# turian/inverse-audio-synthesis

Hardware: AMD Instinct MI355X
Metric: audio-seconds rendered+lossed/sec (whole node), batch=128 4s@44.1kHz (higher is better)
Workload: dtype f32; 1 GPU; BASELINE configs[1]: torchsynth-style Voice render + PQMF(3) analysis + mel-L1 loss, batch 128 x 4 s @ 44100 Hz per GPU; batch_per_gpu=128, samples_per_voice=176400, launch=hipgraph, streams=5, pipelined=True

## Files before the change

inverse-audio-synthesis_amd/csrc/voice_kernels.hip:

```cpp
#include <cstdio>
#include <cstdlib>
#include "voice_math.h"
#include "wave_ops.h"
#include "voice_trig.h"
#include "voice_table.h"

#define VOICE_THREADS 256
#define VOICE_WAVES (VOICE_THREADS / 64)
#define AUDIO_THREADS 256
#define AUDIO_WAVES (AUDIO_THREADS / 64)
#define VOICE_SPT 16
#define VOICE_TILE (AUDIO_THREADS * VOICE_SPT)

__constant__ IasParamRange c_param_table[IAS_NPARAMS] = IAS_PARAM_TABLE_INIT;


__device__ __forceinline__ float mapped_param(const float* __restrict__ params01, int b, int idx) {
  const IasParamRange r = c_param_table[idx];
  return ias_map_param(params01[(size_t)b * IAS_NPARAMS + idx], (float)r.lo, (float)r.span, (float)r.curve,
                       r.symmetric);
}

__device__ __forceinline__ int adsr_base(int a) {
  switch (a) {
// ... 133 lines not shown
  __shared__ float s_head[12];
  __shared__ float s_mode[2][8];
  __shared__ double s_wtot[2][CTLF_LFO_WAVES];
  const int b = blockIdx.x, tid = threadIdx.x, lane = tid & 63, wave = tid >> 6;
  const float eps = (float)IAS_EPS;

  for (int i = tid; i < IAS_CTL_TAB_DOUBLES; i += CTLF_THREADS) s_tab[i] = g_ctl_tab[i];
  if (tid < IAS_NPARAMS) s_p[tid] = mapped_param(params01, b, tid);
  __syncthreads();
  const float note_on = s_p[IAS_P_KEYBOARD_DURATION];
  if (wave == CTLF_WAVES - 1) {
    if (lane < 12) {
      const int a = lane >> 1;
      const float* q = s_p + adsr_base(a);
      IasAdsr e; e.attack = q[0]; e.decay = q[1]; e.sustain = q[2]; e.release = q[3]; e.alpha = q[4];
      const IasAdsrHeads h = ias_adsr_heads(e, note_on, control_rate, eps, s_tab);
      s_head[lane] = (lane & 1) ? h.release_head : h.decay_head;
    }
  } else if (wave == CTLF_WAVES - 2) {
    if (lane < 16 && (lane & 7) < 5) {
      const int l = lane >> 3, k = lane & 7;
      const int qbase = (l == 0) ? IAS_P_LFO_1_FREQUENCY : IAS_P_LFO_2_FREQUENCY;
      s_mode[l][k] = ias_pow_ctl(s_p[qbase + 3 + k], IAS_LFO_EXPONENT_F, s_tab);
    }
  } else if (wave == CTLF_WAVES - 3) {
    if (lane == 0) {
      const float* p = s_p;
      const float midi_f0 = p[IAS_P_KEYBOARD_MIDI_F0];
      IasVoiceConst vc;
      vc.f0_1 = ias_add(midi_f0, p[IAS_P_VCO_1_TUNING]);
      vc.depth_1 = p[IAS_P_VCO_1_MOD_DEPTH];
      vc.phi_1 = p[IAS_P_VCO_1_INITIAL_PHASE];
      vc.f0_2 = ias_add(midi_f0, p[IAS_P_VCO_2_TUNING]);
      vc.depth_2 = p[IAS_P_VCO_2_MOD_DEPTH];
      vc.phi_2 = p[IAS_P_VCO_2_INITIAL_PHASE];
      vc.kpart = ias_partials_k(midi_f0, vc.depth_2);
      vc.shape = p[IAS_P_VCO_2_SHAPE];
      vc.shape_gain = ias_sub(1.0f, ias_div(vc.shape, 2.0f));
      vc.lvl0 = p[IAS_P_MIXER_VCO_1];
      vc.lvl1 = p[IAS_P_MIXER_VCO_2];
      vc.lvl2 = p[IAS_P_MIXER_NOISE];
      vc.pad[0] = vc.pad[1] = vc.pad[2] = vc.pad[3] = 0.0f;
      vconst[b] = vc;
    }
  }
  __syncthreads();

  float* gsig = sig + (size_t)b * 8 * Tc;
  for (int idx = tid; idx < 6 * Tc; idx += CTLF_THREADS) {
    const int slot = idx / Tc, t = idx - slot * Tc;
    const int a = slot < 4 ? slot + 2 : slot - 4;
    const float* q = s_p + adsr_base(a);
    IasAdsr e; e.attack = q[0]; e.decay = q[1]; e.sustain = q[2]; e.release = q[3]; e.alpha = q[4];
    IasAdsrHeads heads; heads.decay_head = s_head[2 * a]; heads.release_head = s_head[2 * a + 1];
    const float v = ias_adsr_headed(t, e, note_on, control_rate, eps, heads, s_tab);
    s_row[a * Tc + t] = v;
    gsig[a * Tc + t] = v;
  }
  if (tid < 2) {
    float* m = s_mode[tid];
    const float sm = (float)((double)m[0] + (double)m[1] + (double)m[2] + (double)m[3] + (double)m[4]);
    for (int k = 0; k < 5; ++k) m[k] = ias_div(m[k], sm);
  }
  __syncthreads();

  {
    const int l = wave / CTLF_LFO_WAVES, w = wave - l * CTLF_LFO_WAVES;
    const int qbase = (l == 0) ? IAS_P_LFO_1_FREQUENCY : IAS_P_LFO_2_FREQUENCY;
    const float freq = s_p[qbase], depth = s_p[qbase + 1], phi = s_p[qbase + 2];
    const float* rate_env = s_row + (4 + l) * Tc;
    const float* amp_env = s_row + (2 + l) * Tc;
    double* sums = s_sum + (size_t)l * Tc;
    const int per_wave = ((Tc + CTLF_LFO_WAVES - 1) / CTLF_LFO_WAVES + 63) / 64 * 64;
    const int t_begin = min(w * per_wave, Tc), t_end = min(t_begin + per_wave, Tc);
    double carry = 0.0;
    for (int t0 = t_begin; t0 < t_end; t0 += 64) {
      const int t = t0 + lane;
      double inc = 0.0;
      if (t < t_end) inc = (double)ias_lfo_inc(freq, depth, rate_env[t], control_rate);
      const double sc = wave_incl_scan(inc, lane) + carry;
      carry = __shfl(sc, 63, 64);
      if (t < t_end) sums[t] = sc;
    }
    if (lane == 0) s_wtot[l][w] = carry;
    __syncthreads();
    double base = 0.0;
    for (int k = 0; k < w; ++k) base += s_wtot[l][k];
    float mode[5];
#pragma unroll
    for (int k = 0; k < 5; ++k) mode[k] = s_mode[l][k];
    for (int t = t_begin + lane; t < t_end; t += 64) {
      const double ph = base + sums[t];
      const float arg = ias_add((float)ph, phi);
      const float o = ias_mul(ias_lfo_shape_mix(arg, mode, s_tab), amp_env[t]);
      s_row[(6 + l) * Tc + t] = o;
      gsig[(6 + l) * Tc + t] = o;
      if (dbg != nullptr) {
        dbg[((size_t)b * 10 + 6 + l) * Tc + t] = arg;
        dbg[((size_t)b * 10 + 8 + l) * Tc + t] = o;
      }
    }
  }
  __syncthreads();

  float* out = ctrl + (size_t)b * IAS_NCTRL * Tc;
  const float* wm = s_p + IAS_P_MOD_MATRIX_ADSR_1_TO_VCO_1_PITCH;
  for (int t = tid; t < Tc; t += CTLF_THREADS) {
    const float e0 = s_row[t], e1 = s_row[Tc + t], l0 = s_row[6 * Tc + t], l1 = s_row[7 * Tc + t];
#pragma unroll
    for (int j = 0; j < IAS_NCTRL; ++j)
      out[j * Tc + t] = ias_dot4_cr(wm[j], wm[5 + j], wm[10 + j], wm[15 + j], e0, e1, l0, l1);
    if (dbg != nullptr) {
#pragma unroll
      for (int r = 0; r < 6; ++r) dbg[((size_t)b * 10 + r) * Tc + t] = s_row[r * Tc + t];
    }
  }
}
static size_t voice_control_fused_lds(int Tc) {
  return sizeof(double) * (IAS_CTL_TAB_DOUBLES + 2 * (size_t)Tc) + sizeof(float) * 8 * (size_t)Tc;
}

#endif

#define VOICE_MAXCTRL 320
#define VOICE_SPIN_LIMIT (1u << 24)
#ifndef VOICE_SPIN_SLEEP
#define VOICE_SPIN_SLEEP 8
#endif
#define VOICE_READY_BIT 0x8000000000000000ull
#ifndef VOICE_MIN_WAVES
#define VOICE_MIN_WAVES 3
#endif
#ifndef VOICE_GROUP
#define VOICE_GROUP 4
#endif
#ifndef VOICE_NCOUNTERS
#define VOICE_NCOUNTERS 8
#endif
#define VOICE_SYNC_HEAD_BYTES ((VOICE_NCOUNTERS + 1) * 128)
#define VOICE_MATH_CR 0
#define VOICE_TAB_DOUBLES ((IAS_EXP2_TAB_LEN + 1) / 2 * 2)
#define VOICE_MATH_HW 1

typedef __attribute__((address_space(1))) unsigned long long gu64;
typedef __attribute__((address_space(1))) unsigned int gu32;

__device__ const double g_exp2_tab[IAS_EXP2_TAB_LEN] = IAS_EXP2_TAB_INIT;

#ifdef VOICE_STAMPS
__device__ unsigned long long* g_voice_stamps = nullptr;
extern "C" int ias_voice_debug_set_stamps(unsigned long long* p) {
  return hipMemcpyToSymbol(HIP_SYMBOL(g_voice_stamps), &p, sizeof(p)) == hipSuccess ? 0 : -3;
}
#define VSTAMP(slot) do { if (g_voice_stamps && have_cur && lane == 0) { unsigned long long* sp_ = g_voice_stamps + ((size_t)(cur.b * ntiles + cur.tile) * 4 + wave) * 12; sp_[slot] = __builtin_amdgcn_s_memtime(); if ((slot) == 0) sp_[10] = __builtin_amdgcn_s_memrealtime(); if ((slot) == 6) sp_[11] = __builtin_amdgcn_s_memrealtime(); } } while (0)
#else
#define VSTAMP(slot) do {} while (0)
#endif

typedef __attribute__((address_space(3))) void voice_lds_void;
typedef const __attribute__((address_space(3))) char voice_lds_cchar;
typedef float voice_f2 __attribute__((ext_vector_type(2)));
typedef const __attribute__((address_space(3))) voice_f2 voice_lds_cfloat2;
typedef const __attribute__((address_space(3))) double voice_lds_cdouble;

__device__ __forceinline__ float voice_exp2_cr_lds(float t, unsigned tab_biased) {
  const float u = fmaf(t, 256.0f, 12582912.0f);
  const float mf = u - 12582912.0f;
  const float r = fmaf(mf, -0.00390625f, t);
  const double tv = *(voice_lds_cdouble*)(uintptr_t)(tab_biased + ((unsigned)__float_as_uint(u) << 3));
  const double rd = (double)r;
  double p = IAS_EXP2_C4;
  p = fma(p, rd, IAS_EXP2_C3);
  p = fma(p, rd, IAS_EXP2_C2);
  p = fma(p, rd, IAS_EXP2_C1);
  p = fma(p, rd, 1.0);
  return (float)(p * tv);
}
typedef const __attribute__((address_space(1))) void voice_glb_void;
__device__ __forceinline__ voice_lds_cchar* voice_ctrl_row(float real, unsigned ctrl_biased) {
  unsigned addr;
  const int k = (int)real;
  asm("v_mad_u32_u24 %0, %1, 40, %2" : "=v"(addr) : "v"(k), "s"(ctrl_biased));
  return (voice_lds_cchar*)(uintptr_t)addr;
}
static_assert(IAS_NCTRL * 8 == 40, "voice_ctrl_row: the row stride is an immediate");
__device__ __forceinline__ float voice_lerp(float w0, float w1, voice_f2 q) { return fmaf(w0, q.x, w1 * q.y); }
template <int MATH, bool FMA_DIV>
__device__ __forceinline__ float voice_inc(float f0, float depth, float pm, unsigned tab_biased, double inv_sample_rate,
                                           float sr_f, float sr_r) {
  float c = f0 + depth * pm;
  c = fminf(fmaxf(c, 0.0f), 127.0f);
  const float t = ias_div_fma(c - 69.0f, 12.0f, 1.0f / 12.0f);
  const float e = (MATH == VOICE_MATH_CR) ? voice_exp2_cr_lds(t, tab_biased) : __builtin_amdgcn_exp2f(t);
  const float w = (float)IAS_TWO_PI_D * (440.0f * e);
  return FMA_DIV ? ias_div_fma(w, sr_f, sr_r) : ias_div_by_recip(w, inv_sample_rate);
}

#define VOICE_CTRL_ROW (IAS_NCTRL * 8)

__device__ __forceinline__ int voice_take_ticket(unsigned int* counters, int& c, int& tried, int ntiles, int nvoices) {
  while (tried < VOICE_NCOUNTERS) {
    const int nv_c = (nvoices - c + VOICE_NCOUNTERS - 1) / VOICE_NCOUNTERS;
    const unsigned n = __hip_atomic_fetch_add((gu32*)(counters + c * 32), 1u, __ATOMIC_RELAXED, __HIP_MEMORY_SCOPE_AGENT);
    if ((int)n < nv_c * ntiles) return (c << 24) | (int)n;
    c = (c + 1) % VOICE_NCOUNTERS;
    ++tried;
  }
  return -1;
}
struct VoiceTile {
  int tile, b, j_tile, c_lo, ncp;
  bool fast;
};
__device__ __forceinline__ VoiceTile voice_tile_of(int ticket, int nvoices, int T, int Tc, float scale) {
  VoiceTile t;
  const int c = ticket >> 24, n = ticket & 0xffffff;
  const int nv_c = (nvoices - c + VOICE_NCOUNTERS - 1) / VOICE_NCOUNTERS;
  t.tile = n / nv_c;
  t.b = (n - t.tile * nv_c) * VOICE_NCOUNTERS + c;
  t.j_tile = t.tile * VOICE_TILE;
  const int j_last = min(t.j_tile + VOICE_TILE, T) - 1;
  int i0, i1; float w0, w1;
  ias_interp_pos(t.j_tile, scale, Tc, i0, i1, w0, w1);
  t.c_lo = i0;
  ias_interp_pos(j_last, scale, Tc, i0, i1, w0, w1);
  t.ncp = i1 - t.c_lo + 1;
  t.fast = (t.j_tile + VOICE_TILE <= T) && (T & 3) == 0;
  return t;
}
__device__ __forceinline__ void voice_stage_ctrl(char* dst, const float* __restrict__ ctrl, const VoiceTile& t, int Tc) {
  const float* cb = ctrl + (size_t)t.b * IAS_NCTRL * Tc;
  for (int i = threadIdx.x; i < IAS_NCTRL * t.ncp; i += AUDIO_THREADS) {
    const int k = i / t.ncp, c = i - k * t.ncp;
    const float* crow = cb + k * Tc;
    reinterpret_cast<float2*>(dst)[c * IAS_NCTRL + k] = make_float2(crow[t.c_lo + c], crow[min(t.c_lo + c + 1, Tc - 1)]);
  }
}

template <int MATH, bool FMA_DIV, bool FAST>
__device__ __forceinline__ void voice_phase_a(const char* s_ctrl, const double* s_tab_, const IasVoiceConst& vc,
                                              const VoiceTile& t, int T, double inv_sample_rate, float sr_f, float sr_r,
                                              float scale, float (&inc1)[VOICE_SPT], float (&inc2)[VOICE_SPT],
                                              double& ex1, double& ex2, double (*wsum)[AUDIO_WAVES]) {
  const int tid = threadIdx.x, lane = tid & 63, wave = tid >> 6;
  const int j0 = t.j_tile + tid * VOICE_SPT;
  const float jf0 = (float)j0;
  const unsigned ctrl_biased = (unsigned)(uintptr_t)(voice_lds_cchar*)s_ctrl - (unsigned)(t.c_lo * VOICE_CTRL_ROW);
  const unsigned s_tab = (unsigned)(uintptr_t)(voice_lds_cchar*)s_tab_ - (0x4B400000u + (unsigned)IAS_EXP2_TAB_MIN) * 8u;
  double tot1 = 0.0, tot2 = 0.0;
#pragma unroll
  for (int e = 0; e < VOICE_SPT; ++e) {
    const float real = scale * (jf0 + (float)e);
    const float w1 = __builtin_amdgcn_fractf(real), w0 = 1.0f - w1;
    voice_lds_cchar* cp = voice_ctrl_row(real, ctrl_biased);
    const voice_f2 q1 = *(voice_lds_cfloat2*)cp, q2 = *(voice_lds_cfloat2*)(cp + 16);
    const float pm1 = voice_lerp(w0, w1, q1), pm2 = voice_lerp(w0, w1, q2);
    float a = voice_inc<MATH, FMA_DIV>(vc.f0_1, vc.depth_1, pm1, s_tab, inv_sample_rate, sr_f, sr_r);
    float d = voice_inc<MATH, FMA_DIV>(vc.f0_2, vc.depth_2, pm2, s_tab, inv_sample_rate, sr_f, sr_r);
    if (!FAST && j0 + e >= T) { a = 0.0f; d = 0.0f; }
    inc1[e] = a; inc2[e] = d;
    tot1 += (double)a; tot2 += (double)d;
    if ((e & (VOICE_GROUP - 1)) == VOICE_GROUP - 1) __builtin_amdgcn_sched_barrier(0);
  }
  const double in1 = wave_incl_scan(tot1, lane), in2 = wave_incl_scan(tot2, lane);
  if (lane == 63) { wsum[0][wave] = in1; wsum[1][wave] = in2; }
  ex1 = in1 - tot1; ex2 = in2 - tot2;
}

template <bool FAST>
__device__ __forceinline__ void voice_phase_b(const char* s_ctrl, float* s_stage, const IasVoiceConst& vc, const VoiceTile& t,
                                              const float* __restrict__ nrow, float* __restrict__ arow, int T, float scale,
                                              const float (&inc1)[VOICE_SPT], const float (&inc2)[VOICE_SPT], double ex1,
                                              double ex2, const double* s_carry, const double (*wsum)[AUDIO_WAVES],
                                              float& pk) {
  const int tid = threadIdx.x, lane = tid & 63;
  const int wave_u = __builtin_amdgcn_readfirstlane(tid >> 6);
  const int j0 = t.j_tile + tid * VOICE_SPT;
  float jf0 = (float)j0;
  asm volatile("" : "+v"(jf0));
  float* stage = s_stage + wave_u * (64 * VOICE_SPT);
  const int j_wave = t.j_tile + wave_u * (64 * VOICE_SPT);
  const int perm = (lane >> 2) & 3;
  const unsigned ctrl_biased = (unsigned)(uintptr_t)(voice_lds_cchar*)s_ctrl - (unsigned)(t.c_lo * VOICE_CTRL_ROW);

  const float kexp = -1.4426950408889634f * vc.kpart;
  double run1 = s_carry[0] + ex1, run2 = s_carry[1] + ex2;
  for (int w = 0; w < wave_u; ++w) { run1 += wsum[0][w]; run2 += wsum[1][w]; }
  float o[4], nz[4];
  float4 nz_next = make_float4(0.f, 0.f, 0.f, 0.f);
  auto load_noise4 = [&](int jq) -> float4 {
    return make_float4(jq < T ? nrow[jq] : 0.0f, jq + 1 < T ? nrow[jq + 1] : 0.0f, jq + 2 < T ? nrow[jq + 2] : 0.0f,
                       jq + 3 < T ? nrow[jq + 3] : 0.0f);
  };
  if (!FAST) nz_next = load_noise4(j0);
#pragma unroll
  for (int e = 0; e < VOICE_SPT; ++e) {
    if ((e & 3) == 0) {
      if (FAST) {
        const float4 v = *reinterpret_cast<const float4*>(stage + lane * VOICE_SPT + 4 * ((e >> 2) ^ perm));
        nz[0] = v.x; nz[1] = v.y; nz[2] = v.z; nz[3] = v.w;
      } else {
        nz[0] = nz_next.x; nz[1] = nz_next.y; nz[2] = nz_next.z; nz[3] = nz_next.w;
        if (e + 4 < VOICE_SPT) nz_next = load_noise4(j0 + e + 4);
      }
    }
    const float real = scale * (jf0 + (float)e);
    const float w1 = __builtin_amdgcn_fractf(real);
    voice_lds_cchar* cp = voice_ctrl_row(real, ctrl_biased);
    const voice_f2 qa = *(voice_lds_cfloat2*)(cp + 8), qb = *(voice_lds_cfloat2*)(cp + 24), qn = *(voice_lds_cfloat2*)(cp + 32);
    const float amp1 = fmaf(w1, qa.y, qa.x), amp2 = fmaf(w1, qb.y, qb.x), ampn = fmaf(w1, qn.y, qn.x);
    run1 += (double)inc1[e]; run2 += (double)inc2[e];
    const float arg1 = (float)run1 + vc.phi_1, arg2 = (float)run2 + vc.phi_2;
    float s2, c2, sgn;
    voice_sincos_sgn(arg2, s2, c2, sgn);
    const float th = voice_tanh_half_of_exp2arg(kexp * s2);
    const float v2 = th * fmaf(vc.shape, c2, sgn);
    float om = voice_cos(arg1) * amp1;
    om = fmaf(v2, amp2, om);
    om = fmaf(nz[e & 3], ampn, om);
    if (FAST || j0 + e < T) pk = fmaxf(pk, fabsf(om));
    o[e & 3] = om;
    if ((e & 3) == 3) {
      if (FAST) {
        *reinterpret_cast<float4*>(stage + lane * VOICE_SPT + 4 * ((e >> 2) ^ perm)) = make_float4(o[0], o[1], o[2], o[3]);
      } else {
        const int jq = j0 + e - 3;
#pragma unroll
        for (int x = 0; x < 4; ++x) if (jq + x < T) arow[jq + x] = o[x];
      }
      if ((e & (VOICE_GROUP - 1)) == VOICE_GROUP - 1) __builtin_amdgcn_sched_barrier(0);
    }
  }
  if (FAST) {
    const int dst = 4 * (lane ^ (lane >> 4));
#pragma unroll
    for (int q = 0; q < VOICE_SPT / 4; ++q)
      *reinterpret_cast<float4*>(arow + j_wave + q * 256 + dst) = *reinterpret_cast<const float4*>(stage + q * 256 + lane * 4);
  }
}

__device__ __forceinline__ float2 voice_ctrl_elem(const float* __restrict__ ctrl, const VoiceTile& t, int Tc, int i) {
  const int k = i / t.ncp, c = i - k * t.ncp;
  const float* crow = ctrl + ((size_t)t.b * IAS_NCTRL + k) * Tc;
  return make_float2(crow[t.c_lo + c], crow[min(t.c_lo + c + 1, Tc - 1)]);
}
__device__ __forceinline__ void voice_ctrl_put(char* dst, const VoiceTile& t, int i, float2 v, const IasVoiceConst& vc) {
  const int k = i / t.ncp, c = i - k * t.ncp;
  if (k == 1 || k == 3 || k == 4) {
    const float g = k == 1 ? vc.lvl0 : (k == 3 ? vc.lvl1 * vc.shape_gain : vc.lvl2);
    const float a = g * v.x;
    v = make_float2(a, g * v.y - a);
  }
  reinterpret_cast<float2*>(dst)[c * IAS_NCTRL + k] = v;
}

#define VOICE_WAVE_LOOKBACK (AUDIO_WAVES - 1)
#define VOICE_WAVE_PUBLISH (AUDIO_WAVES - 2)
template <int MATH, bool FMA_DIV>
__global__ __launch_bounds__(AUDIO_THREADS, VOICE_MIN_WAVES) __attribute__((amdgpu_num_vgpr(76))) void voice_audio_kernel(
    const float* __restrict__ ctrl, const IasVoiceConst* __restrict__ vconst,
    const float* __restrict__ noise, float* __restrict__ audio, unsigned long long* agg ,
    unsigned int* ticket_status ,
    unsigned* __restrict__ rowpeak, int T, int Tc, int ntiles, int nvoices, double inv_sample_rate, float sr_f,
    float sr_r, float scale, int maxctrl) {
  extern __shared__ __attribute__((aligned(16))) double dyn_smem_d[];
  double* s_tab = dyn_smem_d;
  float* s_stage = reinterpret_cast<float*>(dyn_smem_d + VOICE_TAB_DOUBLES);
  char* s_ctrl0 = reinterpret_cast<char*>(s_stage + VOICE_TILE);
  const int ctrl_bytes = maxctrl * VOICE_CTRL_ROW;
  __shared__ double s_wsum[2][2][AUDIO_WAVES];
  __shared__ double s_carry[2];
  __shared__ float s_max[AUDIO_WAVES];
  __shared__ int s_ticket;

  const int tid = threadIdx.x, lane = tid & 63, wave = tid >> 6;
  int my_counter = blockIdx.x % VOICE_NCOUNTERS, counters_tried = 0;
  if (tid == 0) s_ticket = voice_take_ticket(ticket_status, my_counter, counters_tried, ntiles, nvoices);
  if (MATH == VOICE_MATH_CR)
    for (int i = tid; i < IAS_EXP2_TAB_LEN; i += AUDIO_THREADS) s_tab[i] = g_exp2_tab[i];
  __syncthreads();

  VoiceTile cur = {}, next = {};
  bool have_cur = false;
  bool have_next = __builtin_amdgcn_readfirstlane(s_ticket) >= 0;
  float2 pre = make_float2(0.f, 0.f);
  if (have_next) {
    next = voice_tile_of(__builtin_amdgcn_readfirstlane(s_ticket), nvoices, T, Tc, scale);
    if (tid < IAS_NCTRL * next.ncp) pre = voice_ctrl_elem(ctrl, next, Tc, tid);
  }
  int slot = 0;
  float incC1[VOICE_SPT], incC2[VOICE_SPT];
  float incN1[VOICE_SPT], incN2[VOICE_SPT];
  double exC1 = 0.0, exC2 = 0.0, exN1 = 0.0, exN2 = 0.0;
#pragma unroll
  for (int e = 0; e < VOICE_SPT; ++e) { incC1[e] = incC2[e] = 0.0f; }

  while (have_cur || have_next) {
    gu64* row = (gu64*)(agg + ((size_t)cur.b * ntiles) * 2);
    VSTAMP(0);
    if (have_next) {
      char* dst = s_ctrl0 + (slot ^ 1) * ctrl_bytes;
      const IasVoiceConst vcp = vconst[next.b];
      if (tid < IAS_NCTRL * next.ncp) voice_ctrl_put(dst, next, tid, pre, vcp);
      for (int i = tid + AUDIO_THREADS; i < IAS_NCTRL * next.ncp; i += AUDIO_THREADS)
        voice_ctrl_put(dst, next, i, voice_ctrl_elem(ctrl, next, Tc, i), vcp);
    }
    unsigned long long early1 = VOICE_READY_BIT, early2 = VOICE_READY_BIT;
    if (have_cur) {
      if (wave == VOICE_WAVE_LOOKBACK && lane < cur.tile) {
        early1 = __hip_atomic_load(row + lane * 2, __ATOMIC_RELAXED, __HIP_MEMORY_SCOPE_AGENT);
        early2 = __hip_atomic_load(row + lane * 2 + 1, __ATOMIC_RELAXED, __HIP_MEMORY_SCOPE_AGENT);
      }
      if (cur.fast) {
        const int wave_u = __builtin_amdgcn_readfirstlane(wave);
        const float* nsrc = noise + (size_t)cur.b * T + cur.j_tile + wave_u * (64 * VOICE_SPT) + 4 * (lane ^ (lane >> 4));
#pragma unroll
        for (int q = 0; q < VOICE_SPT / 4; ++q)
          __builtin_amdgcn_global_load_lds((voice_glb_void*)(nsrc + q * 256),
                                           (voice_lds_void*)(s_stage + wave_u * (64 * VOICE_SPT) + q * 256), 16, 0, 0);
      }
    }
    __syncthreads();
    VSTAMP(1);
    unsigned after_raw = 0;
    int after_c = 0;
    if (have_next) {
      if (tid == 0) {
        after_c = my_counter;
        after_raw = __hip_atomic_fetch_add((gu32*)(ticket_status + after_c * 32), 1u, __ATOMIC_RELAXED, __HIP_MEMORY_SCOPE_AGENT);
      }
      const IasVoiceConst vcn = vconst[next.b];
#ifdef VOICE_SKIP_A
      if (false)
#else
      if (next.fast)
#endif
        voice_phase_a<MATH, FMA_DIV, true>(s_ctrl0 + (slot ^ 1) * ctrl_bytes, s_tab, vcn, next, T, inv_sample_rate, sr_f, sr_r,
                                           scale, incN1, incN2, exN1, exN2, s_wsum[slot ^ 1]);
#ifndef VOICE_ANALYZE_FULL_ONLY
      else
        voice_phase_a<MATH, FMA_DIV, false>(s_ctrl0 + (slot ^ 1) * ctrl_bytes, s_tab, vcn, next, T, inv_sample_rate, sr_f, sr_r,
                                            scale, incN1, incN2, exN1, exN2, s_wsum[slot ^ 1]);
#endif
      if (tid == 0) {
        const int nv_c = (nvoices - after_c + VOICE_NCOUNTERS - 1) / VOICE_NCOUNTERS;
        int tk = (after_c << 24) | (int)after_raw;
        if ((int)after_raw >= nv_c * ntiles) {
          my_counter = (my_counter + 1) % VOICE_NCOUNTERS;
          ++counters_tried;
          tk = voice_take_ticket(ticket_status, my_counter, counters_tried, ntiles, nvoices);
        }
        s_ticket = tk;
      }
    } else if (tid == 0) {
      s_ticket = -1;
    }
    VSTAMP(2);
    if (have_cur && wave == VOICE_WAVE_LOOKBACK) {
      double a1 = 0.0, a2 = 0.0;
      bool timeout = false;
      for (int t0 = 0; t0 < cur.tile; t0 += 64) {
        const int t = t0 + lane;
        unsigned long long x1 = VOICE_READY_BIT, x2 = VOICE_READY_BIT;
        if (t0 == 0) { x1 = early1; x2 = early2; }
        else if (t < cur.tile) { x1 = 0; x2 = 0; }
        unsigned spins = 0;
        bool ok = (x1 & x2 & VOICE_READY_BIT) != 0;
        while (!__all(ok)) {
          if (++spins > VOICE_SPIN_LIMIT) { timeout = true; break; }
          if (!ok) {
            x1 = __hip_atomic_load(row + t * 2, __ATOMIC_RELAXED, __HIP_MEMORY_SCOPE_AGENT);
            x2 = __hip_atomic_load(row + t * 2 + 1, __ATOMIC_RELAXED, __HIP_MEMORY_SCOPE_AGENT);
            ok = (x1 & x2 & VOICE_READY_BIT) != 0;
          }
          if (!__all(ok)) __builtin_amdgcn_s_sleep(VOICE_SPIN_SLEEP);
        }
        if (t < cur.tile) {
          a1 += __longlong_as_double((long long)(x1 & ~VOICE_READY_BIT));
          a2 += __longlong_as_double((long long)(x2 & ~VOICE_READY_BIT));
        }
      }
      a1 = wave_sum(a1); a2 = wave_sum(a2);
      if (lane == 0) {
        if (timeout) {
          a1 = a2 = __longlong_as_double(0x7ff8000000000000ll);
          __hip_atomic_store((gu32*)ticket_status + VOICE_NCOUNTERS * 32, 1u, __ATOMIC_RELAXED, __HIP_MEMORY_SCOPE_AGENT);
          __hip_atomic_store((gu32*)ticket_status - 32, 1u, __ATOMIC_RELAXED, __HIP_MEMORY_SCOPE_AGENT);
        }
        s_carry[0] = a1; s_carry[1] = a2;
      }
    }
    VSTAMP(3);
    __syncthreads();
    VSTAMP(4);
    if (have_next && wave == VOICE_WAVE_PUBLISH && lane < 2) {
      double a = 0.0;
      for (int w = 0; w < AUDIO_WAVES; ++w) a += s_wsum[slot ^ 1][lane][w];
      gu64* nrow_agg = (gu64*)(agg + ((size_t)next.b * ntiles) * 2);
      __hip_atomic_store(nrow_agg + next.tile * 2 + lane, (unsigned long long)__double_as_longlong(a) | VOICE_READY_BIT,
                         __ATOMIC_RELAXED, __HIP_MEMORY_SCOPE_AGENT);
    }
    const int t_after = __builtin_amdgcn_readfirstlane(s_ticket);
    const bool have_after = t_after >= 0;
    VoiceTile after = {};
    if (have_after) {
      after = voice_tile_of(t_after, nvoices, T, Tc, scale);
      if (tid < IAS_NCTRL * after.ncp) pre = voice_ctrl_elem(ctrl, after, Tc, tid);
    }
    if (have_cur) {
      const IasVoiceConst vc = vconst[cur.b];
      float pk = 0.0f;
#ifdef VOICE_SKIP_B
      if (false)
#else
      if (cur.fast)
#endif
        voice_phase_b<true>(s_ctrl0 + slot * ctrl_bytes, s_stage, vc, cur, noise + (size_t)cur.b * T, audio + (size_t)cur.b * T,
                            T, scale, incC1, incC2, exC1, exC2, s_carry, s_wsum[slot], pk);
#ifndef VOICE_ANALYZE_FULL_ONLY
      else
        voice_phase_b<false>(s_ctrl0 + slot * ctrl_bytes, s_stage, vc, cur, noise + (size_t)cur.b * T, audio + (size_t)cur.b * T,
                             T, scale, incC1, incC2, exC1, exC2, s_carry, s_wsum[slot], pk);
#endif
      pk = wave_max(pk);
      if (lane == 0) s_max[wave] = pk;
    }
    VSTAMP(5);
    __syncthreads();
    VSTAMP(6);
    if (have_cur && tid == 0) {
      float m = s_max[0];
      for (int w = 1; w < AUDIO_WAVES; ++w) m = fmaxf(m, s_max[w]);
      atomicMax(rowpeak + cur.b, __float_as_uint(m));
    }
    cur = next;
    have_cur = have_next;
    next = after;
    have_next = have_after;
    slot ^= 1;
#pragma unroll
    for (int e = 0; e < VOICE_SPT; ++e) { incC1[e] = incN1[e]; incC2[e] = incN2[e]; }
    exC1 = exN1; exC2 = exN2;
  }
}

__global__ __launch_bounds__(256) void voice_normalize_kernel(float* __restrict__ audio,
                                                              const unsigned* __restrict__ rowpeak,
                                                              int T, int nvec_per_row) {
  const int b = blockIdx.y;
  const float peak = __uint_as_float(rowpeak[b]);
  if (!(peak > 1.0f)) return;
  float* row = audio + (size_t)b * T;
  if ((T & 3) == 0) {
    float4* r4 = reinterpret_cast<float4*>(row);
    for (int i = blockIdx.x * blockDim.x + threadIdx.x; i < nvec_per_row; i += gridDim.x * blockDim.x) {
      float4 v = r4[i];
      v.x = ias_div(v.x, peak); v.y = ias_div(v.y, peak);
      v.z = ias_div(v.z, peak); v.w = ias_div(v.w, peak);
      r4[i] = v;
    }
  } else {
    for (int i = blockIdx.x * blockDim.x + threadIdx.x; i < T; i += gridDim.x * blockDim.x)
      row[i] = ias_div(row[i], peak);
  }
}

static inline size_t align_up(size_t x, size_t a) { return (x + a - 1) / a * a; }

struct VoiceWs {
  size_t off_ctrl, off_vconst, off_env, off_sticky, off_sync, sync_bytes, off_agg, off_peak, total;
  int ntiles;
};
static VoiceWs voice_ws_layout(int B, int T, int Tc) {
  VoiceWs w;
  w.ntiles = (T + VOICE_TILE - 1) / VOICE_TILE;
  size_t o = 0;
  w.off_ctrl = o;    o = align_up(o + sizeof(float) * (size_t)B * IAS_NCTRL * Tc, 256);
  w.off_vconst = o;  o = align_up(o + sizeof(IasVoiceConst) * (size_t)B, 256);
  w.off_env = o;     o = align_up(o + sizeof(float) * (size_t)B * 8 * Tc, 256);
  w.off_sticky = o;  o += 128;
  w.off_sync = o;
  w.off_agg = o + VOICE_SYNC_HEAD_BYTES;
  w.off_peak = w.off_agg + sizeof(unsigned long long) * (size_t)B * 2 * w.ntiles;
  w.sync_bytes = align_up(w.off_peak + sizeof(unsigned) * (size_t)B - w.off_sync, 16);
  o = align_up(w.off_sync + w.sync_bytes, 256);
  w.total = o;
  return w;
}

extern "C" long long ias_voice_workspace_bytes(int B, int T, int Tc) {
  if (B <= 0 || T <= 0 || Tc <= 1) return IAS_ERR_ARG;
  return (long long)voice_ws_layout(B, T, Tc).total;
}

static int voice_maxctrl(int T, int Tc) {
  return (int)((double)VOICE_TILE * (double)(Tc - 1) / (double)(T - 1)) + 6;
}

static int voice_check_dims(int B, int T, int Tc) {
  if (B <= 0 || T <= 1 || Tc <= 1 || B > 65535) return IAS_ERR_ARG;
  const double span = (double)VOICE_TILE * (double)(Tc - 1) / (double)(T - 1);
  if (span + 6.0 > (double)VOICE_MAXCTRL) return IAS_ERR_UNSUPPORTED;
  return IAS_OK;
}

bool ias_voice_control_slim_ok(int Tc, int control_rate);
int ias_voice_control_slim_launch(const float* params01, float* ctrl, void* vconst, float* sig, float* dbg, int B, int Tc,
                                  int control_rate, hipStream_t stream);

static int voice_control_launch(const float* params01, float* ctrl, void* vconst, float* sig, float* dbg, int B,
                                int Tc, int control_rate, void* stream_) {
  hipStream_t stream = (hipStream_t)stream_;
  if (!params01 || !ctrl || !vconst || !sig || B <= 0 || B > 65535 || Tc <= 1 || control_rate <= 0) return IAS_ERR_ARG;
  const char* form = ias_diag_env("IAS_VOICE_CTRL");
  if (form == nullptr && ias_voice_control_slim_ok(Tc, control_rate))
    return ias_voice_control_slim_launch(params01, ctrl, vconst, sig, dbg, B, Tc, control_rate, stream);
#ifdef IAS_DIAG
  const size_t flds = voice_control_fused_lds(Tc);
  if (flds <= 156 * 1024 && form != nullptr && form[0] == 'f') {
    static bool attr_set = false;
    if (!attr_set) {
      if (hipFuncSetAttribute((const void*)voice_control_fused_kernel, hipFuncAttributeMaxDynamicSharedMemorySize, 156 * 1024) != hipSuccess)
        return IAS_ERR_LAUNCH;
      attr_set = true;
    }
    hipLaunchKernelGGL(voice_control_fused_kernel, dim3(B), dim3(CTLF_THREADS), flds, stream, params01, sig, ctrl,
                       (IasVoiceConst*)vconst, dbg, Tc, (float)control_rate);
    return hipGetLastError() == hipSuccess ? IAS_OK : IAS_ERR_LAUNCH;
  }
#endif
  const size_t lds = sizeof(double) * (VOICE_WAVES + (size_t)Tc);
  if (lds > 160 * 1024) return IAS_ERR_UNSUPPORTED;
  hipLaunchKernelGGL(voice_env_kernel, dim3(6, B), dim3(VOICE_THREADS), 0, stream, params01, sig, Tc,
                     (float)control_rate);
  if (lds > 64 * 1024)
    (void)hipFuncSetAttribute((const void*)voice_lfo_kernel, hipFuncAttributeMaxDynamicSharedMemorySize, (int)lds);
  hipLaunchKernelGGL(voice_lfo_kernel, dim3(2, B), dim3(VOICE_THREADS), lds, stream, params01, sig, dbg, Tc,
                     (float)control_rate);
  hipLaunchKernelGGL(voice_modmix_kernel, dim3((Tc + VOICE_THREADS - 1) / VOICE_THREADS, B), dim3(VOICE_THREADS), 0,
                     stream, params01, sig, ctrl, (IasVoiceConst*)vconst, dbg, Tc);
  return hipGetLastError() == hipSuccess ? IAS_OK : IAS_ERR_LAUNCH;
}

extern "C" int ias_voice_control(const float* params01, float* ctrl, void* vconst, float* env, float* dbg, int B, int Tc,
                                 int control_rate, void* stream_) {
  return voice_control_launch(params01, ctrl, vconst, env, dbg, B, Tc, control_rate, stream_);
}

extern "C" int ias_voice_control_ws(const float* params01, void* workspace, long long workspace_bytes, int B, int T,
                                    int Tc, int control_rate, void* stream_) {
  if (!workspace) return IAS_ERR_ARG;
  int rc = voice_check_dims(B, T, Tc);
  if (rc) return rc;
  const VoiceWs w = voice_ws_layout(B, T, Tc);
  if ((size_t)workspace_bytes < w.total) return IAS_ERR_WORKSPACE;
  char* ws = (char*)workspace;
  return voice_control_launch(params01, (float*)(ws + w.off_ctrl), ws + w.off_vconst, (float*)(ws + w.off_env), nullptr,
                              B, Tc, control_rate, stream_);
}

template <int MATH, bool FMA_DIV>
static int voice_audio_grid(size_t lds, int total_tiles) {
  static int cached_lds = -1, cached_grid = 0;
  if (cached_lds != (int)lds) {
    int dev = 0, ncu = 256, per_cu = 0;
    (void)hipGetDevice(&dev);
    (void)hipDeviceGetAttribute(&ncu, hipDeviceAttributeMultiprocessorCount, dev);
    if (hipOccupancyMaxActiveBlocksPerMultiprocessor(&per_cu, voice_audio_kernel<MATH, FMA_DIV>, AUDIO_THREADS, lds) != hipSuccess ||
        per_cu < 1)
      per_cu = 2;
    if (const char* e = ias_diag_env("IAS_VOICE_PERCU")) {
      const int v = atoi(e);
      if (v >= 1 && v < per_cu) per_cu = v;
    }
    cached_grid = per_cu * ncu;
    cached_lds = (int)lds;
    if (ias_diag_env("IAS_DEBUG")) fprintf(stderr, "[ias] voice_audio_kernel: %d workgroups/CU x %d CUs, %zu B LDS\n", per_cu, ncu, lds);
  }
  return cached_grid < total_tiles ? cached_grid : total_tiles;
}

template <int MATH, bool FMA_DIV>
static void voice_audio_launch(hipStream_t stream, const VoiceWs& w, char* ws, const float* noise, float* audio, int B,
                               int T, int Tc, int sample_rate) {
  const float scale = (float)(Tc - 1) / (float)(T - 1);
  const float sr_f = (float)sample_rate;
  const int maxctrl = voice_maxctrl(T, Tc);
  const size_t lds = sizeof(double) * VOICE_TAB_DOUBLES + sizeof(float) * VOICE_TILE + 2 * sizeof(float2) * IAS_NCTRL * (size_t)maxctrl;
  if (lds > 64 * 1024)
    (void)hipFuncSetAttribute((const void*)voice_audio_kernel<MATH, FMA_DIV>, hipFuncAttributeMaxDynamicSharedMemorySize, (int)lds);
  const int ntiles = w.ntiles;
  const int grid = voice_audio_grid<MATH, FMA_DIV>(lds, ntiles * B);
  hipLaunchKernelGGL((voice_audio_kernel<MATH, FMA_DIV>), dim3(grid), dim3(AUDIO_THREADS), lds, stream,
                     (const float*)(ws + w.off_ctrl), (const IasVoiceConst*)(ws + w.off_vconst), noise, audio,
                     (unsigned long long*)(ws + w.off_agg), (unsigned int*)(ws + w.off_sync),
                     (unsigned*)(ws + w.off_peak), T, Tc, ntiles, B, 1.0 / (double)sample_rate, sr_f,
                     1.0f / sr_f, scale, maxctrl);
}

extern "C" int ias_voice_stage(int stage, int math_mode, const float* noise, float* audio, void* workspace,
                               long long workspace_bytes, int B, int T, int Tc, int sample_rate, void* stream_) {
  hipStream_t stream = (hipStream_t)stream_;
  if (!workspace || sample_rate <= 0 || stage < 0 || stage > 3 || math_mode < 0 || math_mode > 1) return IAS_ERR_ARG;
  if (stage != 2 && (!noise || !audio)) return IAS_ERR_ARG;
  int rc = voice_check_dims(B, T, Tc);
  if (rc) return rc;
  const VoiceWs w = voice_ws_layout(B, T, Tc);
  if ((size_t)workspace_bytes < w.total) return IAS_ERR_WORKSPACE;
  char* ws = (char*)workspace;
  if (stage == 2) {
    if (hipMemsetAsync(ws + w.off_sync, 0, w.sync_bytes, stream) != hipSuccess) return IAS_ERR_LAUNCH;
  } else if (stage == 0 || stage == 3) {
    if (stage == 0 && hipMemsetAsync(ws + w.off_sync, 0, w.sync_bytes, stream) != hipSuccess) return IAS_ERR_LAUNCH;
    const bool fma_div = ias_div_fma_rate_ok(sample_rate) != 0;
    if (math_mode == VOICE_MATH_CR) {
      if (fma_div) voice_audio_launch<VOICE_MATH_CR, true>(stream, w, ws, noise, audio, B, T, Tc, sample_rate);
      else voice_audio_launch<VOICE_MATH_CR, false>(stream, w, ws, noise, audio, B, T, Tc, sample_rate);
    } else {
      if (fma_div) voice_audio_launch<VOICE_MATH_HW, true>(stream, w, ws, noise, audio, B, T, Tc, sample_rate);
      else voice_audio_launch<VOICE_MATH_HW, false>(stream, w, ws, noise, audio, B, T, Tc, sample_rate);
    }
  } else {
    const int nvec = T / 4;
    int gx = (nvec + 255) / 256;
    if (gx > 64) gx = 64;
    if (gx < 1) gx = 1;
    hipLaunchKernelGGL(voice_normalize_kernel, dim3(gx, B), dim3(256), 0, stream, audio, (unsigned*)(ws + w.off_peak), T,
                       nvec);
  }
  return hipGetLastError() == hipSuccess ? IAS_OK : IAS_ERR_LAUNCH;
}

extern "C" int ias_voice_render(const float* params01, const float* noise, float* audio, void* workspace,
                                long long workspace_bytes, int B, int T, int Tc, int sample_rate,
                                int control_rate, int normalize, int math_mode, void* stream_) {
  if (!params01 || !noise || !audio || !workspace || sample_rate <= 0 || control_rate <= 0) return IAS_ERR_ARG;
  int rc = voice_check_dims(B, T, Tc);
  if (rc) return rc;
  const VoiceWs w = voice_ws_layout(B, T, Tc);
  if ((size_t)workspace_bytes < w.total) return IAS_ERR_WORKSPACE;
  char* ws = (char*)workspace;
  rc = ias_voice_control(params01, (float*)(ws + w.off_ctrl), ws + w.off_vconst, (float*)(ws + w.off_env), nullptr, B,
                         Tc, control_rate, stream_);
  for (int stage = 0; stage < (normalize ? 2 : 1) && rc == IAS_OK; ++stage)
    rc = ias_voice_stage(stage, math_mode, noise, audio, workspace, workspace_bytes, B, T, Tc, sample_rate, stream_);
  return rc;
}

extern "C" int ias_voice_read_status(const void* workspace, unsigned* status_dev, int B, int T, int Tc, void* stream_) {
  if (!workspace || !status_dev) return IAS_ERR_ARG;
  const VoiceWs w = voice_ws_layout(B, T, Tc);
  if (hipMemcpyAsync(status_dev, (const char*)workspace + w.off_sync + VOICE_NCOUNTERS * 128, sizeof(unsigned), hipMemcpyDeviceToDevice,
                     (hipStream_t)stream_) != hipSuccess)
    return IAS_ERR_LAUNCH;
  return IAS_OK;
}

extern "C" int ias_voice_read_status_sticky(void* workspace, unsigned* status_dev, int B, int T, int Tc, int clear,
                                            void* stream_) {
  if (!workspace || !status_dev) return IAS_ERR_ARG;
  const VoiceWs w = voice_ws_layout(B, T, Tc);
  char* word = (char*)workspace + w.off_sticky;
  if (hipMemcpyAsync(status_dev, word, sizeof(unsigned), hipMemcpyDeviceToDevice, (hipStream_t)stream_) != hipSuccess)
    return IAS_ERR_LAUNCH;
  if (clear && hipMemsetAsync(word, 0, sizeof(unsigned), (hipStream_t)stream_) != hipSuccess) return IAS_ERR_LAUNCH;
  return IAS_OK;
}

extern "C" long long ias_voice_ctrl_offset(int B, int T, int Tc) {
  if (B <= 0 || T <= 0 || Tc <= 1) return IAS_ERR_ARG;
  return (long long)voice_ws_layout(B, T, Tc).off_ctrl;
}
extern "C" long long ias_voice_vconst_offset(int B, int T, int Tc) {
  if (B <= 0 || T <= 0 || Tc <= 1) return IAS_ERR_ARG;
  return (long long)voice_ws_layout(B, T, Tc).off_vconst;
}

extern "C" long long ias_voice_peaks_offset(int B, int T, int Tc) {
  if (B <= 0 || T <= 0 || Tc <= 1) return IAS_ERR_ARG;
  return (long long)voice_ws_layout(B, T, Tc).off_peak;
}

__global__ __launch_bounds__(256) void voice_save_kernel(const float* __restrict__ ctrl, const float* __restrict__ vconst,
                                                         const float* __restrict__ peak, float* __restrict__ ctrl_out,
                                                         float* __restrict__ vconst_out, float* __restrict__ peaks_out,
                                                         long long nctrl, int nvc, int npk) {
  const long long i = (long long)blockIdx.x * 256 + threadIdx.x;
  if (i < nctrl) ctrl_out[i] = ctrl[i];
  if (i < nvc) vconst_out[i] = vconst[i];
  if (peaks_out && i < npk) peaks_out[i] = peak[i];
}
extern "C" int ias_voice_save_for_backward(const void* workspace, float* ctrl_out, float* vconst_out, float* peaks_out, int B,
                                           int T, int Tc, void* stream_) {
  if (!workspace || !ctrl_out || !vconst_out || B <= 0 || T <= 0 || Tc <= 1) return IAS_ERR_ARG;
  const VoiceWs w = voice_ws_layout(B, T, Tc);
  const char* ws = (const char*)workspace;
  const long long nctrl = (long long)B * IAS_NCTRL * Tc;
  static_assert(sizeof(IasVoiceConst) == 64, "vconst rows are 16 floats");
  const long long nthreads = nctrl > 16LL * B ? nctrl : 16LL * B;
  hipLaunchKernelGGL(voice_save_kernel, dim3((unsigned)((nthreads + 255) / 256)), dim3(256), 0, (hipStream_t)stream_,
                     (const float*)(ws + w.off_ctrl), (const float*)(ws + w.off_vconst), (const float*)(ws + w.off_peak),
                     ctrl_out, vconst_out, peaks_out, nctrl, B * 16, B);
  return hipGetLastError() == hipSuccess ? IAS_OK : IAS_ERR_LAUNCH;
}

extern "C" int ias_voice_read_peaks(const void* workspace, float* peaks_dev, int B, int T, int Tc, void* stream_) {
  if (!workspace || !peaks_dev) return IAS_ERR_ARG;
  const VoiceWs w = voice_ws_layout(B, T, Tc);
  if (hipMemcpyAsync(peaks_dev, (const char*)workspace + w.off_peak, sizeof(float) * (size_t)B,
                     hipMemcpyDeviceToDevice, (hipStream_t)stream_) != hipSuccess)
    return IAS_ERR_LAUNCH;
  return IAS_OK;
}
```

Baseline: 3.187 million audio-s/s.

## Stage control points per wave and drop two block barriers per tile iteration

After: 3.266 million audio-s/s (median of 6 runs). 1.02x the previous value.

```diff
diff --git a/inverse-audio-synthesis_amd/csrc/voice_kernels.hip b/inverse-audio-synthesis_amd/csrc/voice_kernels.hip
--- a/inverse-audio-synthesis_amd/csrc/voice_kernels.hip
+++ b/inverse-audio-synthesis_amd/csrc/voice_kernels.hip
@@ -309,7 +309,7 @@
 extern "C" int ias_voice_debug_set_stamps(unsigned long long* p) {
   return hipMemcpyToSymbol(HIP_SYMBOL(g_voice_stamps), &p, sizeof(p)) == hipSuccess ? 0 : -3;
 }
-#define VSTAMP(slot) do { if (g_voice_stamps && have_cur && lane == 0) { unsigned long long* sp_ = g_voice_stamps + ((size_t)(cur.b * ntiles + cur.tile) * 4 + wave) * 12; sp_[slot] = __builtin_amdgcn_s_memtime(); if ((slot) == 0) sp_[10] = __builtin_amdgcn_s_memrealtime(); if ((slot) == 6) sp_[11] = __builtin_amdgcn_s_memrealtime(); } } while (0)
+#define VSTAMP(slot) do { if (g_voice_stamps && have_cur && lane == 0) { unsigned long long* sp_ = g_voice_stamps + ((size_t)(cur.b * ntiles + cur.tile) * 4 + wave) * 12; sp_[slot] = __builtin_amdgcn_s_memtime(); if ((slot) == 0) sp_[10] = __builtin_amdgcn_s_memrealtime(); if ((slot) == 5) sp_[11] = __builtin_amdgcn_s_memrealtime(); } } while (0)
 #else
 #define VSTAMP(slot) do {} while (0)
 #endif
@@ -369,29 +369,23 @@
   int tile, b, j_tile, c_lo, ncp;
   bool fast;
 };
-__device__ __forceinline__ VoiceTile voice_tile_of(int ticket, int nvoices, int T, int Tc, float scale) {
+#define VOICE_WAVE_SAMPLES (64 * VOICE_SPT)
+__device__ __forceinline__ VoiceTile voice_tile_of(int ticket, int nvoices, int T, int Tc, float scale, int wave_u) {
   VoiceTile t;
   const int c = ticket >> 24, n = ticket & 0xffffff;
   const int nv_c = (nvoices - c + VOICE_NCOUNTERS - 1) / VOICE_NCOUNTERS;
   t.tile = n / nv_c;
   t.b = (n - t.tile * nv_c) * VOICE_NCOUNTERS + c;
   t.j_tile = t.tile * VOICE_TILE;
-  const int j_last = min(t.j_tile + VOICE_TILE, T) - 1;
+  const int j_first = min(t.j_tile + wave_u * VOICE_WAVE_SAMPLES, T - 1);
+  const int j_last = min(t.j_tile + (wave_u + 1) * VOICE_WAVE_SAMPLES, T) - 1;
   int i0, i1; float w0, w1;
-  ias_interp_pos(t.j_tile, scale, Tc, i0, i1, w0, w1);
+  ias_interp_pos(j_first, scale, Tc, i0, i1, w0, w1);
   t.c_lo = i0;
   ias_interp_pos(j_last, scale, Tc, i0, i1, w0, w1);
-  t.ncp = i1 - t.c_lo + 1;
+  t.ncp = i0 - t.c_lo + 1;
   t.fast = (t.j_tile + VOICE_TILE <= T) && (T & 3) == 0;
   return t;
-}
-__device__ __forceinline__ void voice_stage_ctrl(char* dst, const float* __restrict__ ctrl, const VoiceTile& t, int Tc) {
-  const float* cb = ctrl + (size_t)t.b * IAS_NCTRL * Tc;
-  for (int i = threadIdx.x; i < IAS_NCTRL * t.ncp; i += AUDIO_THREADS) {
-    const int k = i / t.ncp, c = i - k * t.ncp;
-    const float* crow = cb + k * Tc;
-    reinterpret_cast<float2*>(dst)[c * IAS_NCTRL + k] = make_float2(crow[t.c_lo + c], crow[min(t.c_lo + c + 1, Tc - 1)]);
-  }
 }
 
 template <int MATH, bool FMA_DIV, bool FAST>
@@ -513,53 +507,64 @@
 
 #define VOICE_WAVE_LOOKBACK (AUDIO_WAVES - 1)
 #define VOICE_WAVE_PUBLISH (AUDIO_WAVES - 2)
+template <int V> struct VoiceSlot { static constexpr int value = V; };
 template <int MATH, bool FMA_DIV>
 __global__ __launch_bounds__(AUDIO_THREADS, VOICE_MIN_WAVES) __attribute__((amdgpu_num_vgpr(76))) void voice_audio_kernel(
     const float* __restrict__ ctrl, const IasVoiceConst* __restrict__ vconst,
     const float* __restrict__ noise, float* __restrict__ audio, unsigned long long* agg ,
     unsigned int* ticket_status ,
     unsigned* __restrict__ rowpeak, int T, int Tc, int ntiles, int nvoices, double inv_sample_rate, float sr_f,
-    float sr_r, float scale, int maxctrl) {
+    float sr_r, float scale, int wave_maxctrl) {
   extern __shared__ __attribute__((aligned(16))) double dyn_smem_d[];
   double* s_tab = dyn_smem_d;
   float* s_stage = reinterpret_cast<float*>(dyn_smem_d + VOICE_TAB_DOUBLES);
-  char* s_ctrl0 = reinterpret_cast<char*>(s_stage + VOICE_TILE);
-  const int ctrl_bytes = maxctrl * VOICE_CTRL_ROW;
-  __shared__ double s_wsum[2][2][AUDIO_WAVES];
-  __shared__ double s_carry[2];
-  __shared__ float s_max[AUDIO_WAVES];
-  __shared__ int s_ticket;
+  const int ctrl_bytes = wave_maxctrl * VOICE_CTRL_ROW;
+  __shared__ double s_wsum[3][2][AUDIO_WAVES];
+  __shared__ double s_carry[2][2];
+  __shared__ float s_max[2][AUDIO_WAVES];
+  __shared__ int s_ticket[2];
 
   const int tid = threadIdx.x, lane = tid & 63, wave = tid >> 6;
+  const int wave_u = __builtin_amdgcn_readfirstlane(wave);
+  char* s_ctrl_w = reinterpret_cast<char*>(s_stage + VOICE_TILE) + wave_u * 2 * ctrl_bytes;
   int my_counter = blockIdx.x % VOICE_NCOUNTERS, counters_tried = 0;
-  if (tid == 0) s_ticket = voice_take_ticket(ticket_status, my_counter, counters_tried, ntiles, nvoices);
+  if (tid == 0) s_ticket[1] = voice_take_ticket(ticket_status, my_counter, counters_tried, ntiles, nvoices);
   if (MATH == VOICE_MATH_CR)
     for (int i = tid; i < IAS_EXP2_TAB_LEN; i += AUDIO_THREADS) s_tab[i] = g_exp2_tab[i];
   __syncthreads();
 
   VoiceTile cur = {}, next = {};
-  bool have_cur = false;
-  bool have_next = __builtin_amdgcn_readfirstlane(s_ticket) >= 0;
+  bool have_cur = false, have_prev = false;
+  int prev_b = 0, prev_slot = 0;
+  bool have_next = __builtin_amdgcn_readfirstlane(s_ticket[1]) >= 0;
   float2 pre = make_float2(0.f, 0.f);
   if (have_next) {
-    next = voice_tile_of(__builtin_amdgcn_readfirstlane(s_ticket), nvoices, T, Tc, scale);
-    if (tid < IAS_NCTRL * next.ncp) pre = voice_ctrl_elem(ctrl, next, Tc, tid);
-  }
-  int slot = 0;
-  float incC1[VOICE_SPT], incC2[VOICE_SPT];
-  float incN1[VOICE_SPT], incN2[VOICE_SPT];
-  double exC1 = 0.0, exC2 = 0.0, exN1 = 0.0, exN2 = 0.0;
-#pragma unroll
-  for (int e = 0; e < VOICE_SPT; ++e) { incC1[e] = incC2[e] = 0.0f; }
-
-  while (have_cur || have_next) {
+    next = voice_tile_of(__builtin_amdgcn_readfirstlane(s_ticket[1]), nvoices, T, Tc, scale, wave_u);
+    if (lane < IAS_NCTRL * next.ncp) pre = voice_ctrl_elem(ctrl, next, Tc, lane);
+  }
+  int q_cur = 2, q_next = 0;
+  float incA1[VOICE_SPT], incA2[VOICE_SPT], incB1[VOICE_SPT], incB2[VOICE_SPT];
+  double exA1 = 0.0, exA2 = 0.0, exB1 = 0.0, exB2 = 0.0;
+#pragma unroll
+  for (int e = 0; e < VOICE_SPT; ++e) { incA1[e] = incA2[e] = 0.0f; }
+
+  auto merge_peak = [&](int b, int sl) {
+    float m = s_max[sl][0];
+    for (int w = 1; w < AUDIO_WAVES; ++w) m = fmaxf(m, s_max[sl][w]);
+    atomicMax(rowpeak + b, __float_as_uint(m));
+  };
+
+  auto iteration = [&](auto slot_c, const float (&incC1)[VOICE_SPT], const float (&incC2)[VOICE_SPT], double exC1, double exC2,
+                       float (&incN1)[VOICE_SPT], float (&incN2)[VOICE_SPT], double& exN1, double& exN2)
+                       __attribute__((always_inline)) {
+    constexpr int slot = decltype(slot_c)::value;
     gu64* row = (gu64*)(agg + ((size_t)cur.b * ntiles) * 2);
     VSTAMP(0);
     if (have_next) {
-      char* dst = s_ctrl0 + (slot ^ 1) * ctrl_bytes;
+      char* dst = s_ctrl_w + (slot ^ 1) * ctrl_bytes;
       const IasVoiceConst vcp = vconst[next.b];
-      if (tid < IAS_NCTRL * next.ncp) voice_ctrl_put(dst, next, tid, pre, vcp);
-      for (int i = tid + AUDIO_THREADS; i < IAS_NCTRL * next.ncp; i += AUDIO_THREADS)
+      if (lane < IAS_NCTRL * next.ncp) voice_ctrl_put(dst, next, lane, pre, vcp);
+      for (int i = lane + 64; i < IAS_NCTRL * next.ncp; i += 64)
         voice_ctrl_put(dst, next, i, voice_ctrl_elem(ctrl, next, Tc, i), vcp);
     }
     unsigned long long early1 = VOICE_READY_BIT, early2 = VOICE_READY_BIT;
@@ -569,15 +574,13 @@
         early2 = __hip_atomic_load(row + lane * 2 + 1, __ATOMIC_RELAXED, __HIP_MEMORY_SCOPE_AGENT);
       }
       if (cur.fast) {
-        const int wave_u = __builtin_amdgcn_readfirstlane(wave);
-        const float* nsrc = noise + (size_t)cur.b * T + cur.j_tile + wave_u * (64 * VOICE_SPT) + 4 * (lane ^ (lane >> 4));
+        const float* nsrc = noise + (size_t)cur.b * T + cur.j_tile + wave_u * VOICE_WAVE_SAMPLES + 4 * (lane ^ (lane >> 4));
 #pragma unroll
         for (int q = 0; q < VOICE_SPT / 4; ++q)
           __builtin_amdgcn_global_load_lds((voice_glb_void*)(nsrc + q * 256),
-                                           (voice_lds_void*)(s_stage + wave_u * (64 * VOICE_SPT) + q * 256), 16, 0, 0);
+                                           (voice_lds_void*)(s_stage + wave_u * VOICE_WAVE_SAMPLES + q * 256), 16, 0, 0);
       }
     }
-    __syncthreads();
     VSTAMP(1);
     unsigned after_raw = 0;
     int after_c = 0;
@@ -592,12 +595,12 @@
 #else
       if (next.fast)
 #endif
-        voice_phase_a<MATH, FMA_DIV, true>(s_ctrl0 + (slot ^ 1) * ctrl_bytes, s_tab, vcn, next, T, inv_sample_rate, sr_f, sr_r,
-                                           scale, incN1, incN2, exN1, exN2, s_wsum[slot ^ 1]);
+        voice_phase_a<MATH, FMA_DIV, true>(s_ctrl_w + (slot ^ 1) * ctrl_bytes, s_tab, vcn, next, T, inv_sample_rate, sr_f, sr_r,
+                                           scale, incN1, incN2, exN1, exN2, s_wsum[q_next]);
 #ifndef VOICE_ANALYZE_FULL_ONLY
       else
-        voice_phase_a<MATH, FMA_DIV, false>(s_ctrl0 + (slot ^ 1) * ctrl_bytes, s_tab, vcn, next, T, inv_sample_rate, sr_f, sr_r,
-                                            scale, incN1, incN2, exN1, exN2, s_wsum[slot ^ 1]);
+        voice_phase_a<MATH, FMA_DIV, false>(s_ctrl_w + (slot ^ 1) * ctrl_bytes, s_tab, vcn, next, T, inv_sample_rate, sr_f, sr_r,
+                                            scale, incN1, incN2, exN1, exN2, s_wsum[q_next]);
 #endif
       if (tid == 0) {
         const int nv_c = (nvoices - after_c + VOICE_NCOUNTERS - 1) / VOICE_NCOUNTERS;
@@ -607,10 +610,10 @@
           ++counters_tried;
           tk = voice_take_ticket(ticket_status, my_counter, counters_tried, ntiles, nvoices);
         }
-        s_ticket = tk;
+        s_ticket[slot] = tk;
       }
     } else if (tid == 0) {
-      s_ticket = -1;
+      s_ticket[slot] = -1;
     }
     VSTAMP(2);
     if (have_cur && wave == VOICE_WAVE_LOOKBACK) {
@@ -644,25 +647,26 @@
           __hip_atomic_store((gu32*)ticket_status + VOICE_NCOUNTERS * 32, 1u, __ATOMIC_RELAXED, __HIP_MEMORY_SCOPE_AGENT);
           __hip_atomic_store((gu32*)ticket_status - 32, 1u, __ATOMIC_RELAXED, __HIP_MEMORY_SCOPE_AGENT);
         }
-        s_carry[0] = a1; s_carry[1] = a2;
+        s_carry[slot][0] = a1; s_carry[slot][1] = a2;
       }
     }
     VSTAMP(3);
     __syncthreads();
     VSTAMP(4);
+    if (have_prev && tid == 0) merge_peak(prev_b, slot ^ 1);
     if (have_next && wave == VOICE_WAVE_PUBLISH && lane < 2) {
       double a = 0.0;
-      for (int w = 0; w < AUDIO_WAVES; ++w) a += s_wsum[slot ^ 1][lane][w];
+      for (int w = 0; w < AUDIO_WAVES; ++w) a += s_wsum[q_next][lane][w];
       gu64* nrow_agg = (gu64*)(agg + ((size_t)next.b * ntiles) * 2);
       __hip_atomic_store(nrow_agg + next.tile * 2 + lane, (unsigned long long)__double_as_longlong(a) | VOICE_READY_BIT,
                          __ATOMIC_RELAXED, __HIP_MEMORY_SCOPE_AGENT);
     }
-    const int t_after = __builtin_amdgcn_readfirstlane(s_ticket);
+    const int t_after = __builtin_amdgcn_readfirstlane(s_ticket[slot]);
     const bool have_after = t_after >= 0;
     VoiceTile after = {};
     if (have_after) {
-      after = voice_tile_of(t_after, nvoices, T, Tc, scale);
-      if (tid < IAS_NCTRL * after.ncp) pre = voice_ctrl_elem(ctrl, after, Tc, tid);
+      after = voice_tile_of(t_after, nvoices, T, Tc, scale, wave_u);
+      if (lane < IAS_NCTRL * after.ncp) pre = voice_ctrl_elem(ctrl, after, Tc, lane);
     }
     if (have_cur) {
       const IasVoiceConst vc = vconst[cur.b];
@@ -672,33 +676,35 @@
 #else
       if (cur.fast)
 #endif
-        voice_phase_b<true>(s_ctrl0 + slot * ctrl_bytes, s_stage, vc, cur, noise + (size_t)cur.b * T, audio + (size_t)cur.b * T,
-                            T, scale, incC1, incC2, exC1, exC2, s_carry, s_wsum[slot], pk);
+        voice_phase_b<true>(s_ctrl_w + slot * ctrl_bytes, s_stage, vc, cur, noise + (size_t)cur.b * T, audio + (size_t)cur.b * T,
+                            T, scale, incC1, incC2, exC1, exC2, s_carry[slot], s_wsum[q_cur], pk);
 #ifndef VOICE_ANALYZE_FULL_ONLY
       else
-        voice_phase_b<false>(s_ctrl0 + slot * ctrl_bytes, s_stage, vc, cur, noise + (size_t)cur.b * T, audio + (size_t)cur.b * T,
-                             T, scale, incC1, incC2, exC1, exC2, s_carry, s_wsum[slot], pk);
+        voice_phase_b<false>(s_ctrl_w + slot * ctrl_bytes, s_stage, vc, cur, noise + (size_t)cur.b * T, audio + (size_t)cur.b * T,
+                             T, scale, incC1, incC2, exC1, exC2, s_carry[slot], s_wsum[q_cur], pk);
 #endif
       pk = wave_max(pk);
-      if (lane == 0) s_max[wave] = pk;
+      if (lane == 0) s_max[slot][wave] = pk;
     }
     VSTAMP(5);
-    __syncthreads();
-    VSTAMP(6);
-    if (have_cur && tid == 0) {
-      float m = s_max[0];
-      for (int w = 1; w < AUDIO_WAVES; ++w) m = fmaxf(m, s_max[w]);
-      atomicMax(rowpeak + cur.b, __float_as_uint(m));
-    }
+    prev_b = cur.b;
+    have_prev = have_cur;
+    prev_slot = slot;
     cur = next;
     have_cur = have_next;
     next = after;
     have_next = have_after;
-    slot ^= 1;
-#pragma unroll
-    for (int e = 0; e < VOICE_SPT; ++e) { incC1[e] = incN1[e]; incC2[e] = incN2[e]; }
-    exC1 = exN1; exC2 = exN2;
-  }
+    q_cur = q_next;
+    q_next = q_next == 2 ? 0 : q_next + 1;
+  };
+
+  while (have_cur || have_next) {
+    iteration(VoiceSlot<0>(), incA1, incA2, exA1, exA2, incB1, incB2, exB1, exB2);
+    if (!(have_cur || have_next)) break;
+    iteration(VoiceSlot<1>(), incB1, incB2, exB1, exB2, incA1, incA2, exA1, exA2);
+  }
+  __syncthreads();
+  if (have_prev && tid == 0) merge_peak(prev_b, prev_slot);
 }
 
 __global__ __launch_bounds__(256) void voice_normalize_kernel(float* __restrict__ audio,
@@ -750,8 +756,8 @@
   return (long long)voice_ws_layout(B, T, Tc).total;
 }
 
-static int voice_maxctrl(int T, int Tc) {
-  return (int)((double)VOICE_TILE * (double)(Tc - 1) / (double)(T - 1)) + 6;
+static int voice_wave_maxctrl(int T, int Tc) {
+  return (int)((double)(VOICE_TILE / AUDIO_WAVES - 1) * (double)(Tc - 1) / (double)(T - 1)) + 4;
 }
 
 static int voice_check_dims(int B, int T, int Tc) {
@@ -842,8 +848,9 @@
                                int T, int Tc, int sample_rate) {
   const float scale = (float)(Tc - 1) / (float)(T - 1);
   const float sr_f = (float)sample_rate;
-  const int maxctrl = voice_maxctrl(T, Tc);
-  const size_t lds = sizeof(double) * VOICE_TAB_DOUBLES + sizeof(float) * VOICE_TILE + 2 * sizeof(float2) * IAS_NCTRL * (size_t)maxctrl;
+  const int wave_maxctrl = voice_wave_maxctrl(T, Tc);
+  const size_t lds = sizeof(double) * VOICE_TAB_DOUBLES + sizeof(float) * VOICE_TILE +
+                     AUDIO_WAVES * 2 * sizeof(float2) * IAS_NCTRL * (size_t)wave_maxctrl;
   if (lds > 64 * 1024)
     (void)hipFuncSetAttribute((const void*)voice_audio_kernel<MATH, FMA_DIV>, hipFuncAttributeMaxDynamicSharedMemorySize, (int)lds);
   const int ntiles = w.ntiles;
@@ -852,7 +859,7 @@
                      (const float*)(ws + w.off_ctrl), (const IasVoiceConst*)(ws + w.off_vconst), noise, audio,
                      (unsigned long long*)(ws + w.off_agg), (unsigned int*)(ws + w.off_sync),
                      (unsigned*)(ws + w.off_peak), T, Tc, ntiles, B, 1.0 / (double)sample_rate, sr_f,
-                     1.0f / sr_f, scale, maxctrl);
+                     1.0f / sr_f, scale, wave_maxctrl);
 }
 
 extern "C" int ias_voice_stage(int stage, int math_mode, const float* noise, float* audio, void* workspace,
```
